# distributed-swarm/agent-tpu

Measured on AMD Instinct MI355X. Metric: classified rows/sec (whole node) map_classify BERT-base at 1/2/4/8 MI355X, higher is better.
Workload: dtype bf16; 1 GPU; model=bert-base, global_batch=1024, seq_len=128, parallelism=dp1, rccl_world_size=1, pg_world_size=1, distinct_devices=True, num_labels=2, topk=2, hipgraph=True, concurrent_batches=2, cu_split=False, weight_bytes=219212032, last_layer_cls_only=True

## Files before the change

agent_tpu_amd/csrc/bindings.cpp:

```cpp
#include <pybind11/numpy.h>
#include <pybind11/pybind11.h>
#include <pybind11/stl.h>

#include <algorithm>
#include <cstring>
#include <memory>
#include <string>
#include <vector>

#include "atpu/comm.h"
#include "atpu/common.h"
#include "atpu/csv.h"
#include "atpu/kernels.h"
#include "atpu/l2_prefetch.h"
#include "atpu/risk_stream.h"
#include "atpu/runtime.h"

namespace py = pybind11;
using namespace atpu;

namespace {

template <typename T>
T* P(uintptr_t p) {
// ... 130 lines not shown
      },
      "fin[m] = (rstd, rstd*mu) from StatsOut partials [slots][M][2]", py::arg("part"), py::arg("slots"),
      py::arg("M"), py::arg("K"), py::arg("eps"), py::arg("fin"), py::arg("stream"));
  m.def("trace_enabled", &trace_enabled, "roctx tracing active (MI355X_TRACE=1 and roctx loadable)");
  m.def("trace_push", [](const std::string& n) { trace_push(n.c_str()); });
  m.def("trace_pop", &trace_pop);
  m.def("trace_mark", [](const std::string& n) { trace_mark(n.c_str()); });
  m.def("gemm_splitk_splits", &gemm_splitk_splits, "split-K factor chosen for an [M,N,K] GEMM");
  m.def(
      "rand_fill",
      [](uintptr_t dst, int64_t n, bool f32, uint64_t seed, uint64_t sid, float scale0, int64_t n0, float scale1,
         uintptr_t stream) { rand_fill(P<void>(dst), n, f32, seed, sid, scale0, n0, scale1, S(stream)); },
      py::arg("dst"), py::arg("n"), py::arg("f32"), py::arg("seed"), py::arg("sid"), py::arg("scale0"), py::arg("n0"),
      py::arg("scale1"), py::arg("stream"), "seeded random init of a device tensor (atpu/rand.h)");
  m.def(
      "rand_fill_host",
      [](uintptr_t dst, int64_t n, bool f32, uint64_t seed, uint64_t sid, float scale0, int64_t n0, float scale1,
         int threads) {
        py::gil_scoped_release nogil;
        rand_fill_host(P<void>(dst), n, f32, seed, sid, scale0, n0, scale1, threads);
      },
      py::arg("dst"), py::arg("n"), py::arg("f32"), py::arg("seed"), py::arg("sid"), py::arg("scale0"), py::arg("n0"),
      py::arg("scale1"), py::arg("threads") = 8, "CPU twin of rand_fill (bit-identical values)");
  m.def("gemv_selected", &gemv_selected, py::arg("M"), py::arg("N"), py::arg("epi"),
        "true when gemm_bf16 runs this [M, N] problem / epilogue on the <= 4-row GEMV");
  m.def("batch_invariant", &batch_invariant, py::arg("set") = -1,
        "batch-invariant kernel selection (ATPU_BATCH_INVARIANT): 1 on, 0 off, -1 reads; returns the current");
  m.def("gemm_force_tile", &gemm_force_tile, py::arg("set") = -1, "GEMM kernel family override: 0 auto, 64, 128, 256");
  m.def("gemm_dec_mode", &gemm_dec_mode, py::arg("set") = -1,
        "skinny-M GEMM path: 1 = 64x64 multi-stage dec kernel, 0 = 128x128 split-K; returns the current");
  m.def("gemm_256_variant", &gemm_256_variant, py::arg("set") = -1,
        "256x256 GEMM schedule: 1 = 256p ping-pong, 3 = 256l persistent full-line epilogue, "
        "4 = 256n full-line + nt stores (default); set >= 0 switches, returns the current");
  m.def("cu_budget", &cu_budget, py::arg("set") = -1,
        "get/set the CU count persistent grids are sized for (0 = the device's; set it to the CU share of "
        "CU-masked streams)");
  m.def("num_cus", &num_cus, "CUs persistent grids are sized for");
  m.def("make_cu_mask_stream", &make_cu_mask_stream, py::arg("first_bit"), py::arg("nbits"),
        "create a HIP stream restricted to CU-mask bits [first_bit, first_bit+nbits) (bit i -> XCD i % 8); "
        "returns the hipStream_t as an int (wrap with torch.cuda.ExternalStream)");
  m.def("attention_persist_mode", &attention_persist_mode, py::arg("set") = -1,
        "packed BERT attention: 1 = persistent prefetching kernel (default), 0 = one item per workgroup");
  m.attr("EPI_BIAS") = static_cast<int>(kEpiBias);
  m.attr("EPI_GELU") = static_cast<int>(kEpiGelu);
  m.attr("EPI_TANH") = static_cast<int>(kEpiTanh);
  m.attr("EPI_RESIDUAL") = static_cast<int>(kEpiResidual);
  m.attr("EPI_RELU") = static_cast<int>(kEpiRelu);
  m.attr("EPI_OUT_F32") = static_cast<int>(kEpiOutF32);
  m.def(
      "cls_attend",
      [](uintptr_t g, uintptr_t fin, uintptr_t U, uintptr_t lens, uintptr_t Z, int B, int seq, int H, int heads,
         uintptr_t stream) {
        cls_attend(P<const bf16>(g), P<const float>(fin), P<const bf16>(U), P<const int32_t>(lens), P<bf16>(Z), B, seq,
                   H, heads, S(stream));
      },
      "[CLS] attention over raw hidden rows (K / V projection re-associated into U and the out-projection)",
      py::arg("g"), py::arg("fin"), py::arg("U"), py::arg("lens"), py::arg("Z"), py::arg("B"), py::arg("S"),
      py::arg("H"), py::arg("heads"), py::arg("stream"));
  m.def("decode_attention", [](uintptr_t q, int ldq, uintptr_t k, uintptr_t v, int ldkv, int seq_stride, int group,
                               uintptr_t lens, uintptr_t step_dev, uintptr_t hist, int hist_stride, uintptr_t bias,
                               int bias_stride, uintptr_t out, int ldo, int rows, int H, float scale, uintptr_t stream,
                               uintptr_t ws) {
    decode_attention(P<const bf16>(q), ldq, P<const bf16>(k), P<const bf16>(v), ldkv, seq_stride, group,
                     P<const int32_t>(lens), P<const int32_t>(step_dev), P<const int32_t>(hist), hist_stride,
                     P<const float>(bias), bias_stride, P<bf16>(out), ldo, rows, H, scale, S(stream), P<float>(ws));
  }, py::arg("q"), py::arg("ldq"), py::arg("k"), py::arg("v"), py::arg("ldkv"), py::arg("seq_stride"), py::arg("group"),
// ... 449 lines not shown
```

agent_tpu_amd/csrc/include/atpu/common.h:

```cpp
#pragma once

#include <hip/hip_runtime.h>

#include <cstdint>
#include <stdexcept>
#include <string>

namespace atpu {

typedef __bf16 bf16;
typedef __bf16 bf16x8 __attribute__((ext_vector_type(8)));
typedef __bf16 bf16x4 __attribute__((ext_vector_type(4)));
typedef float f32x4 __attribute__((ext_vector_type(4)));
typedef float f32x16 __attribute__((ext_vector_type(16)));

constexpr int kWave = 64;

#define ATPU_GLOBAL_AS __attribute__((address_space(1)))
#define ATPU_LDS_AS __attribute__((address_space(3)))

__device__ __forceinline__ void glds16(const void* gsrc, void* lds) {
  __builtin_amdgcn_global_load_lds((const ATPU_GLOBAL_AS void*)gsrc, (ATPU_LDS_AS void*)lds, 16, 0, 0);
}

__device__ __forceinline__ void wait_vmcnt0() { asm volatile("s_waitcnt vmcnt(0)" ::: "memory"); }

template <int CTRL>
__device__ __forceinline__ float dppf(float x) {
  return __int_as_float(__builtin_amdgcn_update_dpp(0, __float_as_int(x), CTRL, 0xF, 0xF, false));
}
constexpr int kDppMirror = 0x140, kDppHalfMirror = 0x141, kDppXor2 = 0x4E, kDppXor1 = 0xB1;

__device__ __forceinline__ float lane_rows_sum(float x);
__device__ __forceinline__ float lane_rows_max(float x);

__device__ __forceinline__ float wave_sum(float v) {
  v = lane_rows_sum(v);
  v += dppf<kDppMirror>(v);
  v += dppf<kDppHalfMirror>(v);
  v += dppf<kDppXor2>(v);
  return v + dppf<kDppXor1>(v);
}

__device__ __forceinline__ float wave_max(float v) {
  v = lane_rows_max(v);
  v = fmaxf(v, dppf<kDppMirror>(v));
  v = fmaxf(v, dppf<kDppHalfMirror>(v));
  v = fmaxf(v, dppf<kDppXor2>(v));
  return fmaxf(v, dppf<kDppXor1>(v));
}

__device__ __forceinline__ float lane_rows_sum(float x) {
  float a, b, c, d;
  asm volatile("v_mov_b32 %0, %2\n\tv_mov_b32 %1, %2\n\ts_nop 1\n\tv_permlane16_swap_b32 %0, %1"
               : "=&v"(a), "=&v"(b) : "v"(x));
// ... 166 lines not shown
    f32x2 phi;
    asm("v_pk_fma_f32 %0, %1, %2, %3 clamp" : "=v"(phi) : "v"(x[e]), "v"(p[e]), "v"(half));
    const f32x2 g = x[e] * phi;
    v[2 * e] = g[0];
    v[2 * e + 1] = g[1];
  }
}

__device__ __forceinline__ float gelu_poly1(float x) {
  constexpr int kDeg = 10;
  constexpr float kQ[kDeg + 1] = {1.536687613e-01f,  -7.178471889e-03f, 4.856055602e-04f, -3.426085095e-05f,
                                  2.347781901e-06f,  -1.526724844e-07f, 8.713541888e-09f, -4.079194205e-10f,
                                  2.366933385e-11f,  -1.725522828e-12f, 5.926992431e-14f};
  constexpr float kH = 1.056250000e+01f;
  const float w = fmaf(x, x, -kH);
  float p = kQ[kDeg];
#pragma unroll
  for (int k = kDeg - 1; k >= 0; --k) p = fmaf(p, w, kQ[k]);
  float phi;
  asm("v_fma_f32 %0, %1, %2, %3 clamp" : "=v"(phi) : "v"(x), "v"(p), "v"(0.5f));
  return x * phi;
}

__device__ __forceinline__ float bf2f(bf16 x) { return static_cast<float>(x); }
__device__ __forceinline__ bf16 f2bf(float x) { return static_cast<bf16>(x); }

typedef __bf16 bf16x2 __attribute__((ext_vector_type(2)));
typedef unsigned u32x4 __attribute__((ext_vector_type(4)));

__device__ __forceinline__ unsigned pack_bf16x2(float lo, float hi) {
  return __builtin_bit_cast(unsigned, bf16x2{f2bf(lo), f2bf(hi)});
}

__device__ __forceinline__ int xcd_remap(int b, int nblocks) {
  const int q = nblocks / 8, r = nblocks % 8, x = b % 8;
  return (x < r ? x * (q + 1) : r * (q + 1) + (x - r) * q) + b / 8;
}

}

#define ATPU_HIP_CHECK(expr)                                                              \
  do {                                                                                    \
    hipError_t _e = (expr);                                                               \
    if (_e != hipSuccess)                                                                 \
      throw std::runtime_error(std::string("HIP error ") + hipGetErrorString(_e) + " at " + \
                               __FILE__ + ":" + std::to_string(__LINE__));                \
  } while (0)

#define ATPU_CHECK(cond, msg)                                                   \
  do {                                                                          \
    if (!(cond)) throw std::invalid_argument(std::string("atpu: ") + (msg));    \
  } while (0)
```

agent_tpu_amd/csrc/include/atpu/kernels.h:

```cpp
#pragma once
#include <vector>

#include <hip/hip_runtime.h>

#include <cstdint>

namespace atpu {

typedef __bf16 bf16;

void rand_fill(void* dst, int64_t n, bool f32, uint64_t seed, uint64_t sid, float scale0, int64_t n0, float scale1,
               hipStream_t stream);

enum GemmEpilogue : int {
  kEpiBias = 1,
  kEpiGelu = 2,
  kEpiTanh = 4,
  kEpiResidual = 8,
  kEpiRelu = 16,
  kEpiOutF32 = 32,
  kEpiInNorm = 64,
  kEpiResNorm = 128,
  kEpiStatsOut = 256,
  kEpiKvScatter = 1024,
// ... 9 lines not shown
  const bf16* Bt = nullptr;
  int ldb = 0;
  bf16* C = nullptr;
  int ldc = 0;
  const float* bias = nullptr;
  const bf16* R = nullptr;
  int ldr = 0;
  int M = 0, N = 0, K = 0;
  int epi = 0;
  int splits = 1;
  float* ws = nullptr;
  const float* in_fin = nullptr;
  const float* colsum = nullptr;
  const float* res_fin = nullptr;
  const float* gamma = nullptr;
  float* part_out = nullptr;
  const float* in_part = nullptr;
  const float* res_part = nullptr;
  float rms_eps = 0.f;
  bf16* kv_cache = nullptr;
  int kv_ld = 0, kv_T = 0, kv_col0 = 0;
  const int32_t* kv_step = nullptr;
  const bf16* pf_w = nullptr;
  int pf_ld = 0, pf_k = 0, pf_n = 0;
  int pf_rpb = 16;
};
void gemm_bf16(const GemmArgs& g, hipStream_t stream);
bool gemv_selected(int M, int N, int epi);
int gemm_splitk_splits(int M, int N, int K);
int gemm_dec_mode(int set);
int batch_invariant(int set);
int gemm_force_tile(int set);
int gemm_256_variant(int set);
void gemm256h(const GemmArgs& g, int mode, hipStream_t stream);
void qkv_attention(const GemmArgs& g, const int32_t* lens, float scale, hipStream_t stream);
void cls_attend(const bf16* g, const float* fin, const bf16* U, const int32_t* lens, bf16* Z, int B, int S, int H,
                int heads, hipStream_t stream);

void quantize_rows_i8(const bf16* x, int ldx, int8_t* q, int ldq, float* scale, int rows, int K,
                      hipStream_t stream);
struct GemmI8Args {
  const int8_t* A = nullptr;
  int lda = 0;
  const float* a_scale = nullptr;
  const int8_t* Bt = nullptr;
  int ldb = 0;
  const float* b_scale = nullptr;
  bf16* C = nullptr;
  int ldc = 0;
  const float* bias = nullptr;
  const bf16* R = nullptr;
  int ldr = 0;
  int M = 0, N = 0, K = 0;
  int epi = 0;
  int32_t* acc_out = nullptr;
  int ldacc = 0;
};
void gemm_i8(const GemmI8Args& g, hipStream_t stream);
bool gemm_i8_ok(int M, int N, int K);
void layernorm_quant_i8(const bf16* x, const bf16* res, const float* gamma, const float* beta, bf16* out, int8_t* q,
                        float* scale, int rows, int N, float eps, hipStream_t stream);

int attention_persist_mode(int set);
int num_cus();
int cu_budget(int set);
int64_t make_cu_mask_stream(int first_bit, int nbits);
// ... 88 lines not shown
```

agent_tpu_amd/csrc/kernels/gemm_bf16.hip:

```cpp
#include "atpu/common.h"
#include "atpu/kernels.h"
#include "atpu/l2_prefetch.h"

#include <hip/hip_ext.h>

#include <algorithm>
#include <cstdlib>
#include <string>
#include <type_traits>

#ifndef ATPU_GEMM_SYNC_EPI
#define ATPU_GEMM_SYNC_EPI 1
#endif

namespace atpu {
namespace {

constexpr int kBK = 64;
constexpr int kRowBytes = kBK * 2;

__device__ __forceinline__ int swz(int row, int chunk) { return chunk ^ ((row >> 1) & 7); }

struct KvOut {
  bf16* cache = nullptr;
// ... 671 lines not shown
      const f32x2 s = f32x2{sum_lane_rows(s1[0] + s1[1]), sum_lane_rows(s2[0] + s2[1])};
      if (fc == 0) *reinterpret_cast<f32x2*>(ln.st + (wn * 256 + lrow) * 2) = s;
    }
#pragma unroll
    for (int j = 0; j < 4; ++j) {
      const unsigned p0 = pack_bf16x2(v[j][0], v[j][1]), p1 = pack_bf16x2(v[j][2], v[j][3]);
      typedef unsigned u32x2 __attribute__((ext_vector_type(2)));
      *reinterpret_cast<u32x2*>(scratch + frag_off(j)) = u32x2{p0, p1};
    }
    const u32x4 o0 = *reinterpret_cast<const u32x4*>(scratch + line_off0);
    const u32x4 o1 = *reinterpret_cast<const u32x4*>(scratch + line_off1);
    u32x4* cp = reinterpret_cast<u32x4*>(C + (row0 + i * 16 + lr) * ldc + col);
    u32x4* cp1 = reinterpret_cast<u32x4*>(C + (row0 + i * 16 + lr + 8) * ldc + col);
    if constexpr (NOST) {
      asm volatile("" ::"v"(o0), "v"(o1), "v"(cp), "v"(cp1));
    } else if constexpr (NT) {
      __builtin_nontemporal_store(o0, cp);
      __builtin_nontemporal_store(o1, cp1);
    } else {
      *cp = o0;
      *cp1 = o1;
    }
  }
}

struct LnFold {
  const float* in_fin;
  const float* colsum;
  const float* res_fin;
  const float* gamma;
  float* part_out;
};

template <int EPI, int DBG = 0, bool NT = false, bool LINE = false>
__global__ __launch_bounds__(512, 1) void gemm256s_kernel(
    const bf16* __restrict__ A, int lda, const bf16* __restrict__ Bt, int ldb, bf16* __restrict__ C, int ldc,
    const float* __restrict__ bias, const bf16* __restrict__ R, int ldr, int M, int N, int K, LnFold lf) {
  using namespace g2;
  constexpr int kImg = 256 * 128;
  constexpr int kEpiOps = kLineBlocks * kLineStoresPerBlock;
  static_assert(kEpiOps == 16, "epilogue store count changed: re-derive the relaxed waits");
  constexpr int kBiasOff = 2 * 2 * kImg;
  constexpr int kEpiOff = kBiasOff + 2 * 256 * 4;
  constexpr bool kIn = EPI & kEpiInNorm, kRes = EPI & kEpiResNorm, kSt = EPI & kEpiStatsOut;
  static_assert(!(kIn || kRes || kSt) || LINE, "LayerNorm folding needs the full-line epilogue");
  static_assert(!(kIn && (kRes || kSt)), "InNorm and ResNorm/StatsOut do not share one kernel (LDS budget)");
  constexpr int kXOff = kEpiOff + (LINE ? 8 * 2048 : 0);
  constexpr int kFinOff = kXOff;
  constexpr int kColOff = kFinOff + (kIn ? 4096 : kRes ? 2048 : 0);
  constexpr int kStOff = kColOff + ((kIn || kRes) ? 1024 : 0);
  constexpr int kLdsBytes = kStOff + (kSt ? 4 * 2048 : 0);
  static_assert(kLdsBytes <= 160 * 1024, "LDS budget");
  __shared__ __attribute__((aligned(16))) char lds[kLdsBytes];
  const int tid = threadIdx.x, lane = tid & 63;
  const int wave = __builtin_amdgcn_readfirstlane(tid >> 6);
  const int ntn = N / 256, ntm = (M + 255) / 256, ntiles = ntm * ntn;
  const int G = gridDim.x;
  const int wm = wave >> 2, wn = wave & 3;
  int v = blockIdx.x;
  if (v >= ntiles) return;

  const int spos = lane & 7;
  auto qrow = [&](int q, int ql) {
    return (q == 0 || q == 3) ? (ql & 63) + (ql >> 6) * 128 + (q == 3 ? 64 : 0)
                              : (ql & 31) + (ql >> 5) * 64 + (q == 2 ? 32 : 0);
  };
  int dst[4][2];
#pragma unroll
  for (int q = 0; q < 4; ++q)
#pragma unroll
    for (int i = 0; i < 2; ++i) dst[q][i] = (q == 0 || q == 3 ? 0 : kImg) + qrow(q, (i * 8 + wave) * 8) * 128;
  auto opaque_lane = [] {
    int l = __lane_id();
    asm volatile("" : "+v"(l));
    return l;
  };
  constexpr bool kFold = kIn || kRes || kSt;
  constexpr bool kSyncEpi = ATPU_GEMM_SYNC_EPI && !(DBG & 128);
  constexpr bool kInAcc = kIn && (DBG & 16);
  constexpr bool kPeel = kRes || kSt || (kIn && !kInAcc);
  constexpr bool kBiasAcc = (kRes || kSt) && (EPI & kEpiBias);
  const bf16* src[4][2];
  uint32_t soff[4][2];
  auto set_src = [&](int tm0, int tn0) {
    const int ln = kFold ? opaque_lane() : lane;
#pragma unroll
    for (int q = 0; q < 4; ++q)
#pragma unroll
      for (int i = 0; i < 2; ++i) {
        const int r = qrow(q, (i * 8 + wave) * 8 + (ln >> 3));
        const size_t e = (q == 0 || q == 3) ? (size_t)min(tm0 + r, M - 1) * lda + sw(r, ln & 7) * 8
                                            : (size_t)(tn0 + r) * ldb + sw(r, ln & 7) * 8;
        if constexpr (kFold) soff[q][i] = (uint32_t)(e * 2);
        else src[q][i] = ((q == 0 || q == 3) ? A : Bt) + e;
      }
  };
  auto stage = [&](int q, int kt, int buf) {
    char* base = lds + buf * 2 * kImg;
    const int koff = kt * 64;
    if constexpr (kFold) {
      const char* g = reinterpret_cast<const char*>((q == 0 || q == 3) ? A : Bt) + koff * 2;
      glds16(g + soff[q][0], base + dst[q][0]);
      glds16(g + soff[q][1], base + dst[q][1]);
    } else {
      glds16(src[q][0] + koff, base + dst[q][0]);
      glds16(src[q][1] + koff, base + dst[q][1]);
    }
  };

  const int fr = lane & 15, fc = lane >> 4;
  f32x4 acc[8][4];
  bf16x8 af[2][4], bl[2][2], br[2][2];
  auto read_a = [&](int buf, int qm) {
    const char* img = lds + buf * 2 * kImg;
#pragma unroll
    for (int ks = 0; ks < 2; ++ks)
#pragma unroll
      for (int i = 0; i < 4; ++i) {
        const int r = wm * 128 + qm * 64 + i * 16 + fr;
        af[ks][i] = *reinterpret_cast<const bf16x8*>(img + r * 128 + sw(r, ks * 4 + fc) * 16);
      }
  };
  auto read_b = [&](bf16x8 (&f)[2][2], int buf, int qn) {
    const char* img = lds + buf * 2 * kImg + kImg;
#pragma unroll
    for (int ks = 0; ks < 2; ++ks)
#pragma unroll
      for (int j = 0; j < 2; ++j) {
        const int r = wn * 64 + qn * 32 + j * 16 + fr;
        f[ks][j] = *reinterpret_cast<const bf16x8*>(img + r * 128 + sw(r, ks * 4 + fc) * 16);
      }
  };
  auto mma = [&](const bf16x8 (&bf)[2][2], int qm, int qn) {
#pragma unroll
    for (int ks = 0; ks < 2; ++ks)
#pragma unroll
// ... 7 lines not shown
  const int nk = K / 64;
  auto glds4 = [&](const float* ubase, char* ldst) {
    const uint32_t lo = (uint32_t)opaque_lane() * 4u;
    __builtin_amdgcn_global_load_lds((const ATPU_GLOBAL_AS void*)(reinterpret_cast<const char*>(ubase) + lo),
                                     (ATPU_LDS_AS void*)ldst, 4, 0, 0);
  };
  auto ln_stage = [&](int tm0, int tn0) {
    if constexpr (kRes || (kIn && !kInAcc)) {
      glds4((kRes ? lf.res_fin : lf.in_fin) + (size_t)tm0 * 2 + wave * 64, lds + kFinOff + wave * 256);
      glds4((kRes ? lf.gamma : lf.colsum) + tn0 + (wave & 3) * 64, lds + kColOff + (wave & 3) * 256);
    }
  };
  auto ln_stage_in = [&](int tm0, int tn0, int par) {
    if constexpr (kInAcc) {
      glds4(lf.in_fin + (size_t)tm0 * 2 + wave * 64, lds + kFinOff + par * 2048 + wave * 256);
      glds4(lf.colsum + tn0 + (wave & 3) * 64, lds + kColOff + (wave & 3) * 256);
    }
  };
  auto ln_flush = [&](int fm0, int fn0) {
    if constexpr (kSt) {
      const int l = opaque_lane();
      if (l < 32) {
        const int r = wave * 32 + l;
        f32x2 s = f32x2{0.f, 0.f};
#pragma unroll
        for (int w = 0; w < 4; ++w) s += *reinterpret_cast<const f32x2*>(lds + kStOff + (w * 256 + r) * 8);
        float* ub = lf.part_out + ((size_t)(fn0 >> 8) * M + fm0 + wave * 32) * 2;
        *reinterpret_cast<f32x2*>(reinterpret_cast<char*>(ub) + (uint32_t)l * 8u) = s;
      }
    }
  };
  int pm0 = 0, pn0 = 0;

  int tile = xcd_remap(v, ntiles);
  int m0 = (tile / ntn) * 256, n0 = (tile % ntn) * 256;
  set_src(m0, n0);
  if constexpr (kBiasAcc) glds4(bias + n0 + (wave & 3) * 64, lds + kBiasOff + (wave & 3) * 256);
  ln_stage_in(m0, n0, 0);
#pragma unroll
  for (int q = 0; q < 4; ++q) stage(q, 0, 0);
  asm volatile("s_waitcnt vmcnt(0)\n\ts_barrier" ::: "memory");
  if (wm == 1) __builtin_amdgcn_s_barrier();
  __builtin_amdgcn_sched_barrier(0);

#define ATPU_PS_SYNC_MMA(BF, QM, QN)                         \
  __builtin_amdgcn_sched_barrier(0);                        \
  __builtin_amdgcn_s_barrier();                             \
  asm volatile("s_waitcnt lgkmcnt(0)" ::: "memory");        \
  __builtin_amdgcn_sched_barrier(0);                        \
  __builtin_amdgcn_s_setprio(1);                            \
  mma(BF, QM, QN);                                          \
  __builtin_amdgcn_s_setprio(0);                            \
  __builtin_amdgcn_sched_barrier(0);                        \
  __builtin_amdgcn_s_barrier();                             \
  __builtin_amdgcn_sched_barrier(0)

  int buf = 0;
  int tile_par = 0;
  bool first = true;
  for (;;) {
    if constexpr (kBiasAcc) {
#pragma unroll
      for (int j = 0; j < 4; ++j) {
        const f32x4 b = *reinterpret_cast<const f32x4*>(lds + kBiasOff + (wn * 64 + j * 16 + fc * 4) * 4);
#pragma unroll
        for (int i = 0; i < 8; ++i) acc[i][j] = b;
      }
    } else if constexpr (kInAcc) {
      const int ol = opaque_lane();
      f32x4 c4[4];
#pragma unroll
      for (int j = 0; j < 4; ++j)
        c4[j] = *reinterpret_cast<const f32x4*>(lds + kColOff + (wn * 64 + j * 16 + (ol >> 4) * 4) * 4);
#pragma unroll
      for (int i = 0; i < 8; ++i) {
        const f32x2 f = *reinterpret_cast<const f32x2*>(lds + kFinOff + tile_par * 2048 +
                                                        (wm * 128 + i * 16 + (ol & 15)) * 8);
        const float nmu = -f[1] * __builtin_amdgcn_rcpf(f[0]);
#pragma unroll
        for (int j = 0; j < 4; ++j) acc[i][j] = c4[j] * nmu;
      }
    } else {
#pragma unroll
      for (int i = 0; i < 8; ++i)
#pragma unroll
        for (int j = 0; j < 4; ++j) acc[i][j] = f32x4{0.f, 0.f, 0.f, 0.f};
    }
    const int vn = v + G;
    const bool has_next = vn < ntiles;
    const int cm0 = m0, cn0 = n0;
    u32x4 pre[2][2];
    auto kstep = [&](int t, auto last_c, auto peel_c) {
      constexpr bool last = decltype(last_c)::value;
      constexpr int P = decltype(peel_c)::value;
      const bool is_t0 = P == -2 ? t == 0 : P == 0;
      const bool more = !last || has_next;
      int kn = t + 1;
      if (last && has_next) {
        tile = xcd_remap(vn, ntiles);
        m0 = (tile / ntn) * 256;
        n0 = (tile % ntn) * 256;
        set_src(m0, n0);
        kn = 0;
      }
      const bool relax = is_t0 && !first;
      read_a(buf, 0);
      read_b(bl, buf, 0);
      if constexpr (kBiasAcc) {
        if (last && has_next) glds4(bias + n0 + (wave & 3) * 64, lds + kBiasOff + (wave & 3) * 256);
      } else if ((EPI & kEpiBias) && is_t0) {
        const int bl_lane = (kIn || kRes || kSt) ? opaque_lane() : lane;
        __builtin_amdgcn_global_load_lds((const ATPU_GLOBAL_AS void*)(bias + cn0 + (wave & 3) * 64 + bl_lane),
                                         (ATPU_LDS_AS void*)(lds + kBiasOff + (tile_par * 256 + (wave & 3) * 64) * 4),
                                         4, 0, 0);
      }
      if constexpr (kInAcc) {
        if (last && has_next) ln_stage_in(m0, n0, tile_par ^ 1);
      }
      if constexpr (kPeel) {
        if constexpr (P == 1) {
          ln_stage(cm0, cn0);
          if (!first) ln_flush(pm0, pn0);
        }
      }
      if (more) {
        stage(0, kn, buf ^ 1);
        if (relax) asm volatile("s_waitcnt vmcnt(%0)" ::"n"(4 + kEpiOps) : "memory");
        else asm volatile("s_waitcnt vmcnt(4)" ::: "memory");
      } else {
        asm volatile("s_waitcnt vmcnt(2)" ::: "memory");
      }
      ATPU_PS_SYNC_MMA(bl, 0, 0);
      read_b(br, buf, 1);
      if (more) {
// ... 42 lines not shown
      for (int t = 0; t + 1 < nk; ++t) kstep(t, std::false_type{}, std::integral_constant<int, -2>{});
      kstep(nk - 1, std::true_type{}, std::integral_constant<int, -2>{});
    }
    if constexpr (kSyncEpi) {
      __builtin_amdgcn_sched_barrier(0);
      if (wm == 0) __builtin_amdgcn_s_barrier();
      __builtin_amdgcn_sched_barrier(0);
    }
    if constexpr (DBG & 1) {
#pragma unroll
      for (int i = 0; i < 8; ++i)
#pragma unroll
        for (int j = 0; j < 4; ++j) asm volatile("" ::"v"(acc[i][j]));
    } else {
      constexpr int kEpiRun0 = kBiasAcc ? (EPI & ~kEpiBias) : EPI;
      constexpr int kEpiRun = (DBG & 8) ? (kEpiRun0 & ~(kEpiInNorm | kEpiResNorm | kEpiStatsOut)) : kEpiRun0;
      if constexpr (LINE)
        epilogue_256_line<kEpiRun, NT, kInAcc, ((DBG >> 5) & 3), bool(DBG & 256)>(
            acc, cm0, cn0, wm, wn, (kIn || kRes || kSt) ? opaque_lane() : lane, C, ldc, R, ldr,
            reinterpret_cast<const float*>(lds + kBiasOff) + tile_par * 256, lds + kEpiOff + wave * 2048, pre,
            LnLds{reinterpret_cast<const float*>(lds + kFinOff + (kInAcc ? tile_par * 2048 : 0)),
                  reinterpret_cast<const float*>(lds + kColOff), reinterpret_cast<float*>(lds + kStOff)});
      else
        epilogue_256<EPI, true, (DBG >> 1), NT>(acc, cm0, cn0, wm, wn, lane, C, ldc, bias, R, ldr, M,
                                            reinterpret_cast<const float*>(lds + kBiasOff) + tile_par * 256);
    }
    if constexpr (kSyncEpi) {
      __builtin_amdgcn_sched_barrier(0);
      if (wm == 1) __builtin_amdgcn_s_barrier();
    }
    pm0 = cm0;
    pn0 = cn0;
    if (!has_next) break;
    v = vn;
    first = false;
    tile_par ^= 1;
  }
#undef ATPU_PS_SYNC_MMA
  if (wm == 0) __builtin_amdgcn_s_barrier();
  if constexpr (kSt) {
    asm volatile("s_waitcnt lgkmcnt(0)" ::: "memory");
    __builtin_amdgcn_s_barrier();
    ln_flush(pm0, pn0);
  }
}


}

static int g_cu_budget = 0;

int cu_budget(int set) {
  if (set >= 0) g_cu_budget = set;
  return g_cu_budget;
}

int num_cus() {
  static const int n = [] {
    int dev = 0, cus = 0;
    if (hipGetDevice(&dev) != hipSuccess || hipDeviceGetAttribute(&cus, hipDeviceAttributeMultiprocessorCount, dev) !=
                                                 hipSuccess)
      cus = 256;
    return cus > 0 ? cus : 256;
  }();
  return g_cu_budget > 0 ? std::min(g_cu_budget, n) : n;
}

int64_t make_cu_mask_stream(int first_bit, int nbits) {
  uint32_t mask[8] = {0, 0, 0, 0, 0, 0, 0, 0};
  for (int b = first_bit; b < first_bit + nbits && b < 256; ++b) mask[b / 32] |= 1u << (b % 32);
  hipStream_t s = nullptr;
  ATPU_HIP_CHECK(hipExtStreamCreateWithCUMask(&s, 8, mask));
  return reinterpret_cast<int64_t>(s);
}

namespace {

template <bool NT, bool LINE = false>
void launch_256s(const GemmArgs& g, hipStream_t s) {
  const int tiles = ((g.M + 255) / 256) * (g.N / 256);
  int nb = std::min(tiles, num_cus());
  if (nb >= 8) nb &= ~7;
  const LnFold lf{g.in_fin, g.colsum, g.res_fin, g.gamma, g.part_out};
#define ATPU_G256S(E)                                                                                          \
  case E:                                                                                                      \
    hipLaunchKernelGGL((gemm256s_kernel<E, 0, NT, LINE>), dim3(nb), dim3(512), 0, s, g.A, g.lda, g.Bt, g.ldb, g.C, g.ldc, \
                       g.bias, g.R, g.ldr, g.M, g.N, g.K, lf);                                                 \
    break;
  if constexpr (LINE) {
    switch (g.epi) {
      ATPU_G256S(kEpiBias | kEpiInNorm)
      ATPU_G256S(kEpiBias | kEpiInNorm | kEpiGelu)
      ATPU_G256S(kEpiBias | kEpiResidual | kEpiStatsOut)
      ATPU_G256S(kEpiBias | kEpiResidual | kEpiResNorm | kEpiStatsOut)
      default:
        break;
    }
    if (g.epi & (kEpiInNorm | kEpiResNorm | kEpiStatsOut)) return;
  }
  switch (g.epi) {
    ATPU_G256S(0)
    ATPU_G256S(kEpiBias)
    ATPU_G256S(kEpiBias | kEpiGelu)
    ATPU_G256S(kEpiBias | kEpiTanh)
    ATPU_G256S(kEpiBias | kEpiResidual)
    ATPU_G256S(kEpiResidual)
    ATPU_G256S(kEpiGelu)
    ATPU_G256S(kEpiRelu)
    default:
      throw std::invalid_argument("atpu: unsupported GEMM epilogue " + std::to_string(g.epi));
  }
#undef ATPU_G256S
}





template <int N>
__device__ __forceinline__ void wait_vmcnt() {
  asm volatile("s_waitcnt vmcnt(%0)" ::"n"(N) : "memory");
}

template <int EPI, int NJ>
__device__ __forceinline__ void dec_row_vals(const f32x4 (&acc)[NJ], int m, int nb, int fchunk, int N, float rstd,
                                             float rmu, float2 rf, bf16* __restrict__ C, int ldc,
                                             const float* __restrict__ bias, const bf16* __restrict__ R, int ldr,
                                             const KvOut& kvo, const LnDec& ln, int kv_pos, bf16x4 (&ov)[NJ]) {
#pragma unroll
  for (int j = 0; j < NJ; ++j) {
    const int n = nb + j * 16 + fchunk * 4;
    if (n >= N) continue;
    f32x4 v = acc[j];
    if constexpr (EPI & kEpiRowRms) v *= rstd;
    if constexpr (EPI & kEpiRowLn) {
      const f32x4 cs = *reinterpret_cast<const f32x4*>(ln.colsum + n);
#pragma unroll
      for (int e = 0; e < 4; ++e) v[e] = fmaf(v[e], rstd, -rmu * cs[e]);
    }
    if constexpr (EPI & kEpiBias) v += *reinterpret_cast<const f32x4*>(bias + n);
    if constexpr (EPI & kEpiGelu) {
#pragma unroll
      for (int e = 0; e < 4; ++e) v[e] = gelu_poly1(v[e]);
    }
    if constexpr (EPI & kEpiTanh) {
// ... 1083 lines not shown
```

agent_tpu_amd/csrc/kernels/qkv_attn.hip:

```cpp
#include "atpu/common.h"
#include "atpu/kernels.h"
#include "atpu/lds_ops.h"

#include <algorithm>

namespace atpu {
namespace {

constexpr int kHImgA = 256 * 128;
constexpr int kHImgB = 192 * 128;
constexpr int kHBuf = kHImgA + kHImgB;
constexpr int kHStores = 24;

__device__ __forceinline__ int hq_row(int q, int ql) {
  switch (q) {
    case 0: return (ql & 63) + (ql >> 6) * 128;
    case 3: return (ql & 63) + (ql >> 6) * 128 + 64;
    case 1: return (ql >> 5) * 48 + (ql & 31);
    default: return (ql >> 4) * 48 + 32 + (ql & 15);
  }
}
constexpr int hq_rounds(int q) { return q == 2 ? 1 : 2; }

constexpr int kAImg = kAttnImg;

template <int EPI, int MODE>
__global__ __launch_bounds__(512, 1) void gemm256h_kernel(const bf16* __restrict__ A, int lda,
                                                          const bf16* __restrict__ Bt, int ldb,
                                                          bf16* __restrict__ C, int ldc,
                                                          const float* __restrict__ bias,
                                                          const float* __restrict__ in_fin,
                                                          const float* __restrict__ colsum, int M, int N, int K,
                                                          const int32_t* __restrict__ lens, float scale) {
  constexpr bool kIn = EPI & kEpiInNorm;
  constexpr int kImgOff = kHBuf;
  constexpr int kBiasOff = MODE == 2 ? kImgOff + 6 * kAImg : 2 * kHBuf;
  constexpr int kFinOff = kBiasOff + 2 * 1024;
  constexpr int kColOff = kFinOff + 2048;
  constexpr int kLds = kColOff + 1024;
  constexpr int kEpiOps = MODE == 0 ? kHStores : MODE == 2 ? 4 : 0;
  constexpr int kLn1 = kIn ? 2 : 0;
  static_assert(kLds <= 160 * 1024, "LDS budget");
  __shared__ __attribute__((aligned(16))) char lds[kLds];
  const int tid = threadIdx.x, lane = tid & 63;
  const int wave = __builtin_amdgcn_readfirstlane(tid >> 6);
  const int wm = wave >> 2, wn = wave & 3;
  const int ntn = N / 192, ntiles = (M / 256) * ntn;
  const int G = gridDim.x;
  int v = blockIdx.x;
  if (v >= ntiles) return;

  auto opaque_lane = [] {
    int l = __lane_id();
    asm volatile("" : "+v"(l));
    return l;
  };
  int dst[4][2];
#pragma unroll
  for (int q = 0; q < 4; ++q)
#pragma unroll
    for (int i = 0; i < 2; ++i)
      dst[q][i] = (q == 0 || q == 3 ? 0 : kHImgA) + hq_row(q, (i * 8 + wave) * 8) * 128;
  uint32_t soff[4][2];
  auto set_src = [&](int tm0, int tn0) {
    const int ln = opaque_lane();
#pragma unroll
    for (int q = 0; q < 4; ++q)
#pragma unroll
      for (int i = 0; i < hq_rounds(q); ++i) {
        const int r = hq_row(q, (i * 8 + wave) * 8 + (ln >> 3));
        const size_t e = (q == 0 || q == 3) ? (size_t)(tm0 + r) * lda + hsw(r, ln & 7) * 8
                                            : (size_t)(tn0 + r) * ldb + hsw(r, ln & 7) * 8;
        soff[q][i] = (uint32_t)(e * 2);
      }
  };
  auto stage = [&](int q, int kt, int buf) {
    char* base = lds + buf * kHBuf;
    const char* g = reinterpret_cast<const char*>((q == 0 || q == 3) ? A : Bt) + kt * 128;
#pragma unroll
    for (int i = 0; i < hq_rounds(q); ++i) glds16(g + soff[q][i], base + dst[q][i]);
  };
  auto glds4 = [&](const float* ubase, int nvalid, char* ldst) {
    const int l = opaque_lane();
    __builtin_amdgcn_global_load_lds((const ATPU_GLOBAL_AS void*)(ubase + min(l, nvalid - 1)),
                                     (ATPU_LDS_AS void*)ldst, 4, 0, 0);
  };

  const int fr = lane & 15, fc = lane >> 4;
  f32x4 acc[8][3];
  bf16x8 af[2][4], b01[2][2], b2[2];
  auto read_a = [&](int buf, int qm) {
    const char* img = lds + buf * kHBuf;
#pragma unroll
    for (int ks = 0; ks < 2; ++ks)
#pragma unroll
      for (int i = 0; i < 4; ++i) {
        const int r = wm * 128 + qm * 64 + i * 16 + fr;
        af[ks][i] = *reinterpret_cast<const bf16x8*>(img + r * 128 + hsw(r, ks * 4 + fc) * 16);
      }
  };
  auto read_b01 = [&](int buf) {
    const char* img = lds + buf * kHBuf + kHImgA;
#pragma unroll
    for (int ks = 0; ks < 2; ++ks)
#pragma unroll
      for (int j = 0; j < 2; ++j) {
        const int r = wn * 48 + j * 16 + fr;
        b01[ks][j] = *reinterpret_cast<const bf16x8*>(img + r * 128 + hsw(r, ks * 4 + fc) * 16);
      }
  };
  auto read_b2 = [&](int buf) {
    const char* img = lds + buf * kHBuf + kHImgA;
#pragma unroll
// ... 168 lines not shown
    for (int ks = 0; ks < 4; ++ks) {
#pragma unroll
      for (int dt = 0; dt < 4; ++dt)
        o[1][dt] = __builtin_amdgcn_mfma_f32_16x16x32_bf16(vfrag(ks, dt), pf[1][ks],
                                                             ks ? o[1][dt] : f32x4{0.f, 0.f, 0.f, 0.f}, 0, 0, 0);
      o[1][4] = __builtin_amdgcn_mfma_f32_16x16x32_bf16(ones, pf[1][ks], ks ? o[1][4] : f32x4{0.f, 0.f, 0.f, 0.f}, 0, 0, 0);
    }
    __builtin_amdgcn_sched_barrier(0);
    char* ost = const_cast<char*>(qi) + wn * 32 * 128;
    const float inv1 = len > 0 && o[1][4][0] > 0.f ? 1.f / o[1][4][0] : 0.f;
#pragma unroll
    for (int dt = 0; dt < 4; ++dt) {
      unsigned x0 = xw[dt][0], x1 = xw[dt][1];
      unsigned y0 = pack_bf16x2(o[1][dt][0] * inv1, o[1][dt][1] * inv1);
      unsigned y1 = pack_bf16x2(o[1][dt][2] * inv1, o[1][dt][3] * inv1);
      swap16(x0, y0);
      swap16(x1, y1);
      const int ro = (fc & 1) * 16 + fr, ch = dt * 2 + (fc >> 1);
      *reinterpret_cast<u32x4*>(ost + ro * 128 + asw(ro, ch) * 16) = u32x4{x0, x1, y0, y1};
    }
    const int l2 = opaque_lane();
    const int lr = l2 >> 3, lc8 = l2 & 7;
    bf16* obase = C + (size_t)(tm0 + wm * 128 + wn * 32 + lr) * ldc + h * 64 + lc8 * 8;
#pragma unroll
    for (int hh = 0; hh < 4; ++hh) {
      const int ro = hh * 8 + lr;
      const u32x4 val = *reinterpret_cast<const u32x4*>(ost + ro * 128 + asw(ro, lc8) * 16);
      u32x4* dst = reinterpret_cast<u32x4*>(obase + (size_t)(hh * 8) * ldc);
      *dst = val;
    }
  };

  const int nk = K / 64;
  int tile = xcd_remap(v, ntiles);
  int m0 = (tile / ntn) * 256, n0 = (tile % ntn) * 192;
  set_src(m0, n0);
#pragma unroll
  for (int q = 0; q < 4; ++q) stage(q, 0, 0);
  asm volatile("s_waitcnt vmcnt(0)\n\ts_barrier" ::: "memory");
  if (wm == 1) __builtin_amdgcn_s_barrier();
  __builtin_amdgcn_sched_barrier(0);

#define ATPU_H_SYNC_MMA(MMA)                                \
  __builtin_amdgcn_sched_barrier(0);                        \
  __builtin_amdgcn_s_barrier();                             \
  asm volatile("s_waitcnt lgkmcnt(0)" ::: "memory");        \
  __builtin_amdgcn_sched_barrier(0);                        \
  __builtin_amdgcn_s_setprio(1);                            \
  MMA;                                                      \
  __builtin_amdgcn_s_setprio(0);                            \
  __builtin_amdgcn_sched_barrier(0);                        \
  __builtin_amdgcn_s_barrier();                             \
  __builtin_amdgcn_sched_barrier(0)

  int buf = 0, tile_par = 0;
  bool first = true;
  for (;;) {
#pragma unroll
    for (int i = 0; i < 8; ++i)
#pragma unroll
      for (int j = 0; j < 3; ++j) acc[i][j] = f32x4{0.f, 0.f, 0.f, 0.f};
    const int vn = v + G;
    const bool has_next = vn < ntiles;
    const int cm0 = m0, cn0 = n0;
    auto kstep = [&](int t, auto last_c, auto peel_c) {
      constexpr bool last = decltype(last_c)::value;
      constexpr int P = decltype(peel_c)::value;
      const bool more = !last || has_next;
      int kn = t + 1;
      if (last && has_next) {
        tile = xcd_remap(vn, ntiles);
        m0 = (tile / ntn) * 256;
        n0 = (tile % ntn) * 192;
        set_src(m0, n0);
        kn = 0;
      }
      const bool relax = P == 0 && !first;
      constexpr int kX = P == 0 ? 1 : (P == 1 ? kLn1 : 0);
      read_a(buf, 0);
      read_b01(buf);
      if (more) {
        stage(0, kn, buf ^ 1);
        stage(1, kn, buf ^ 1);
        if constexpr (P == 0) {
          glds4(bias + cn0 + wn * 48, 48, lds + kBiasOff + tile_par * 1024 + wn * 256);
        }
        if constexpr (P == 1 && kIn) {
          glds4(in_fin + (size_t)cm0 * 2 + wave * 64, 64, lds + kFinOff + wave * 256);
          glds4(colsum + cn0 + wn * 48, 48, lds + kColOff + wn * 256);
        }
        if (relax) asm volatile("s_waitcnt vmcnt(%0)" ::"n"(6 + kEpiOps + kX) : "memory");
        else asm volatile("s_waitcnt vmcnt(%0)" ::"n"(6 + kX) : "memory");
      } else {
        asm volatile("s_waitcnt vmcnt(2)" ::: "memory");
      }
      ATPU_H_SYNC_MMA(mma01(0));
      read_b2(buf);
      if (more) {
        stage(2, kn, buf ^ 1);
        if (relax) asm volatile("s_waitcnt vmcnt(%0)" ::"n"(5 + kEpiOps + kX) : "memory");
        else asm volatile("s_waitcnt vmcnt(%0)" ::"n"(5 + kX) : "memory");
      } else {
        asm volatile("s_waitcnt vmcnt(0)" ::: "memory");
      }
      ATPU_H_SYNC_MMA(mma2(0));
      read_a(buf, 1);
// ... 66 lines not shown
            *reinterpret_cast<u32x2*>(C + (size_t)(cm0 + wm * 128 + i * 16 + ofr) * ldc + cn0 + wn * 48 + j * 16 +
                                      ofc * 4) = u32x2{p0, p1};
          }
        }
      } else {
#pragma unroll
        for (int i = 0; i < 8; i += 2) {
#pragma unroll
          for (int j = 0; j < 3; ++j) {
            unsigned x0, x1, y0, y1;
            frag(i, j, x0, x1);
            frag(i + 1, j, y0, y1);
            swap16(x0, y0);
            swap16(x1, y1);
            const int cb = wn * 48 + j * 16, typ = cb >> 6;
            const int r = (i + (ofc & 1)) * 16 + ofr, ch = ((cb & 63) >> 3) + (ofc >> 1);
            *reinterpret_cast<u32x4*>(lds + kImgOff + (wm * 3 + typ) * kAImg + r * 128 + asw(r, ch) * 16) =
                u32x4{x0, x1, y0, y1};
          }
        }
      }
      if constexpr (MODE == 2) {
        asm volatile("s_waitcnt lgkmcnt(0)" ::: "memory");
        __builtin_amdgcn_s_barrier();
        __builtin_amdgcn_sched_barrier(0);
        attend(cm0, cn0 / 192, len);
        asm volatile("s_waitcnt lgkmcnt(0)" ::: "memory");
        __builtin_amdgcn_s_barrier();
      }
    }
    __builtin_amdgcn_sched_barrier(0);
    if (wm == 1) __builtin_amdgcn_s_barrier();
    if (!has_next) break;
    v = vn;
    first = false;
    tile_par ^= 1;
  }
#undef ATPU_H_SYNC_MMA
  if (wm == 0) __builtin_amdgcn_s_barrier();
}

}

static void launch_256h(const GemmArgs& g, int mode, const int32_t* lens, float scale, hipStream_t s) {
  ATPU_CHECK(g.N % 192 == 0 && g.M % 256 == 0 && g.K % 64 == 0 && g.K >= 256,
             "gemm256h: N % 192, M % 256 == 0, K % 64 == 0 and K >= 256");
  ATPU_CHECK(g.epi == kEpiBias || g.epi == (kEpiBias | kEpiInNorm), "gemm256h: epilogue bias or bias|InNorm");
  ATPU_CHECK(!(g.epi & kEpiInNorm) || (g.in_fin && g.colsum), "gemm256h: InNorm needs in_fin and colsum");
  ATPU_CHECK(g.bias && g.ldc % 4 == 0 && (reinterpret_cast<uintptr_t>(g.C) & 7) == 0, "gemm256h: bias, 8-B rows");
  ATPU_CHECK((size_t)g.M * g.lda * 2 < (1ull << 32) && (size_t)g.N * g.ldb * 2 < (1ull << 32),
             "gemm256h: A and Bt under 4 GiB (32-bit staging offsets)");
  ATPU_CHECK(mode >= 0 && mode <= 2, "gemm256h: mode 0 (store), 1 (timing only) or 2 (attention)");
  if (mode == 2) {
    ATPU_CHECK((g.K / 64) % 2 == 0, "qkv_attention: K / 64 must be even");
    ATPU_CHECK(lens && g.ldc % 8 == 0 && (reinterpret_cast<uintptr_t>(g.C) & 15) == 0,
               "qkv_attention: lens and 16-B aligned context rows");
  }
  const int tiles = (g.M / 256) * (g.N / 192);
  int nb = std::min(tiles, num_cus());
  if (nb >= 8) nb &= ~7;
#define ATPU_GH(E, MD)                                                                                          \
  hipLaunchKernelGGL((gemm256h_kernel<E, MD>), dim3(nb), dim3(512), 0, s, g.A, g.lda, g.Bt, g.ldb, g.C, g.ldc, \
                     g.bias, g.in_fin, g.colsum, g.M, g.N, g.K, lens, scale)
  if (g.epi & kEpiInNorm) {
    if (mode == 0) ATPU_GH(kEpiBias | kEpiInNorm, 0);
    else if (mode == 1) ATPU_GH(kEpiBias | kEpiInNorm, 1);
    else ATPU_GH(kEpiBias | kEpiInNorm, 2);
  } else {
    if (mode == 0) ATPU_GH(kEpiBias, 0);
    else if (mode == 1) ATPU_GH(kEpiBias, 1);
    else ATPU_GH(kEpiBias, 2);
  }
#undef ATPU_GH
  ATPU_HIP_CHECK(hipGetLastError());
}

void gemm256h(const GemmArgs& g, int mode, hipStream_t s) {
  ATPU_CHECK(mode == 0 || mode == 1, "gemm256h: mode 0 (store) or 1 (timing only, no epilogue)");
  launch_256h(g, mode, nullptr, 0.f, s);
}

void qkv_attention(const GemmArgs& g, const int32_t* lens, float scale, hipStream_t s) {
  launch_256h(g, 2, lens, scale, s);
}

}
```

Measured before the change: 52860 rows/s.

## Add XCD column-grouped tile walk and nt A-load policy to persistent GEMMs

Replaces the xcd_remap tile ordering in the persistent 256s and 256h GEMM kernels with a parameterised per-XCD walk. The walk can confine each XCD to a group of weight columns so the weights it reads stay resident in that XCD's L2. It also adds a template cache-policy option for the A-operand LDS-DMA loads (nt) and exposes both through env vars and bindings, plus host tools to inspect the walk. The defaults (cols=1, policy 0) are meant to reproduce the previous xcd_remap ordering with default loads, so the change mainly adds tuning knobs and carries a small cost of extra kernel arguments and index arithmetic.

```diff
diff --git a/agent_tpu_amd/csrc/bindings.cpp b/agent_tpu_amd/csrc/bindings.cpp
--- a/agent_tpu_amd/csrc/bindings.cpp
+++ b/agent_tpu_amd/csrc/bindings.cpp
@@ -186,6 +186,17 @@
   m.def("gemm_256_variant", &gemm_256_variant, py::arg("set") = -1,
         "256x256 GEMM schedule: 1 = 256p ping-pong, 3 = 256l persistent full-line epilogue, "
         "4 = 256n full-line + nt stores (default); set >= 0 switches, returns the current");
+  m.def("gemm_xcd_cols", &gemm_xcd_cols, py::arg("set") = -1,
+        "XCD tile walk of the persistent GEMMs: 0 = auto (column groups from the weight shape), 1 = the xcd_remap "
+        "walk, 2/4/8 = forced column groups; set >= 0 switches, returns the current (ATPU_GEMM_XCD_COLS)");
+  m.def("gemm_a_policy", &gemm_a_policy, py::arg("set") = -1,
+        "A-operand LDS-DMA cache policy of the persistent GEMMs: 0 = default loads, 1 = nt; set >= 0 switches, "
+        "returns the current (ATPU_GEMM_A_POLICY)");
+  m.def("gemm_walk_cols", &gemm_walk_cols, py::arg("ntn"), py::arg("tile_n"), py::arg("K"), py::arg("grid") = -1,
+        "column groups the launcher uses for a weight of ntn column tiles of tile_n rows and depth K "
+        "(1 below 8 workgroups and under cu_budget > 0)");
+  m.def("gemm_tile_walk", &gemm_tile_walk, py::arg("ntm"), py::arg("ntn"), py::arg("grid"), py::arg("cg"),
+        "host view of the persistent tile walk: the tile ids each of `grid` workgroups computes, in order");
   m.def("cu_budget", &cu_budget, py::arg("set") = -1,
         "get/set the CU count persistent grids are sized for (0 = the device's; set it to the CU share of "
         "CU-masked streams)");
diff --git a/agent_tpu_amd/csrc/include/atpu/common.h b/agent_tpu_amd/csrc/include/atpu/common.h
--- a/agent_tpu_amd/csrc/include/atpu/common.h
+++ b/agent_tpu_amd/csrc/include/atpu/common.h
@@ -21,6 +21,11 @@
 
 __device__ __forceinline__ void glds16(const void* gsrc, void* lds) {
   __builtin_amdgcn_global_load_lds((const ATPU_GLOBAL_AS void*)gsrc, (ATPU_LDS_AS void*)lds, 16, 0, 0);
+}
+
+template <int POL>
+__device__ __forceinline__ void glds16_pol(const void* gsrc, void* lds) {
+  __builtin_amdgcn_global_load_lds((const ATPU_GLOBAL_AS void*)gsrc, (ATPU_LDS_AS void*)lds, 16, 0, POL);
 }
 
 __device__ __forceinline__ void wait_vmcnt0() { asm volatile("s_waitcnt vmcnt(0)" ::: "memory"); }
@@ -253,9 +258,32 @@
   return __builtin_bit_cast(unsigned, bf16x2{f2bf(lo), f2bf(hi)});
 }
 
-__device__ __forceinline__ int xcd_remap(int b, int nblocks) {
+__host__ __device__ __forceinline__ int xcd_remap(int b, int nblocks) {
   const int q = nblocks / 8, r = nblocks % 8, x = b % 8;
   return (x < r ? x * (q + 1) : r * (q + 1) + (x - r) * q) + b / 8;
+}
+
+struct XcdWalk {
+  int row0, col0, ncol, off, count;
+};
+
+__host__ __device__ __forceinline__ XcdWalk xcd_walk_init(int x, int ntm, int ntn, int cg) {
+  if (cg <= 1) {
+    const int nt = ntm * ntn, q = nt / 8, r = nt % 8;
+    const int start = x < r ? x * (q + 1) : r * (q + 1) + (x - r) * q;
+    return XcdWalk{start / ntn, 0, ntn, start % ntn, q + (x < r ? 1 : 0)};
+  }
+  const int per = 8 / cg, g = x / per, j = x % per;
+  const int q = ntm / per, r = ntm % per, ncol = ntn / cg;
+  return XcdWalk{j < r ? j * (q + 1) : r * (q + 1) + (j - r) * q, g * ncol, ncol, 0, (q + (j < r ? 1 : 0)) * ncol};
+}
+
+__host__ __device__ __forceinline__ int xcd_col_walk(int v, int ntm, int ntn, int cg) {
+  const XcdWalk w = xcd_walk_init(v % 8, ntm, ntn, cg);
+  const int l = v / 8;
+  if (l >= w.count) return -1;
+  const int p = w.off + l, r = p / w.ncol;
+  return (w.row0 + r) * ntn + w.col0 + (p - r * w.ncol);
 }
 
 }
diff --git a/agent_tpu_amd/csrc/include/atpu/kernels.h b/agent_tpu_amd/csrc/include/atpu/kernels.h
--- a/agent_tpu_amd/csrc/include/atpu/kernels.h
+++ b/agent_tpu_amd/csrc/include/atpu/kernels.h
@@ -65,6 +65,10 @@
 int batch_invariant(int set);
 int gemm_force_tile(int set);
 int gemm_256_variant(int set);
+int gemm_xcd_cols(int set);
+int gemm_a_policy(int set);
+int gemm_walk_cols(int ntn, int tile_n, int K, int grid);
+std::vector<std::vector<int>> gemm_tile_walk(int ntm, int ntn, int grid, int cg);
 void gemm256h(const GemmArgs& g, int mode, hipStream_t stream);
 void qkv_attention(const GemmArgs& g, const int32_t* lens, float scale, hipStream_t stream);
 void cls_attend(const bf16* g, const float* fin, const bf16* U, const int32_t* lens, bf16* Z, int B, int S, int H,
diff --git a/agent_tpu_amd/csrc/kernels/gemm_bf16.hip b/agent_tpu_amd/csrc/kernels/gemm_bf16.hip
--- a/agent_tpu_amd/csrc/kernels/gemm_bf16.hip
+++ b/agent_tpu_amd/csrc/kernels/gemm_bf16.hip
@@ -727,10 +727,10 @@
   float* part_out;
 };
 
-template <int EPI, int DBG = 0, bool NT = false, bool LINE = false>
+template <int EPI, int DBG = 0, bool NT = false, bool LINE = false, int APOL = 0>
 __global__ __launch_bounds__(512, 1) void gemm256s_kernel(
     const bf16* __restrict__ A, int lda, const bf16* __restrict__ Bt, int ldb, bf16* __restrict__ C, int ldc,
-    const float* __restrict__ bias, const bf16* __restrict__ R, int ldr, int M, int N, int K, LnFold lf) {
+    const float* __restrict__ bias, const bf16* __restrict__ R, int ldr, int M, int N, int K, LnFold lf, int cg) {
   using namespace g2;
   constexpr int kImg = 256 * 128;
   constexpr int kEpiOps = kLineBlocks * kLineStoresPerBlock;
@@ -749,11 +749,12 @@
   __shared__ __attribute__((aligned(16))) char lds[kLdsBytes];
   const int tid = threadIdx.x, lane = tid & 63;
   const int wave = __builtin_amdgcn_readfirstlane(tid >> 6);
-  const int ntn = N / 256, ntm = (M + 255) / 256, ntiles = ntm * ntn;
-  const int G = gridDim.x;
+  const int ntn = N / 256, ntm = (M + 255) / 256;
+  const XcdWalk xw = xcd_walk_init(blockIdx.x % 8, ntm, ntn, cg);
+  const int wstep = max((int)gridDim.x / 8, 1);
   const int wm = wave >> 2, wn = wave & 3;
-  int v = blockIdx.x;
-  if (v >= ntiles) return;
+  int wl = blockIdx.x / 8;
+  if (wl >= xw.count) return;
 
   const int spos = lane & 7;
   auto qrow = [&](int q, int ql) {
@@ -795,8 +796,16 @@
     const int koff = kt * 64;
     if constexpr (kFold) {
       const char* g = reinterpret_cast<const char*>((q == 0 || q == 3) ? A : Bt) + koff * 2;
-      glds16(g + soff[q][0], base + dst[q][0]);
-      glds16(g + soff[q][1], base + dst[q][1]);
+      if (q == 0 || q == 3) {
+        glds16_pol<APOL>(g + soff[q][0], base + dst[q][0]);
+        glds16_pol<APOL>(g + soff[q][1], base + dst[q][1]);
+      } else {
+        glds16(g + soff[q][0], base + dst[q][0]);
+        glds16(g + soff[q][1], base + dst[q][1]);
+      }
+    } else if (q == 0 || q == 3) {
+      glds16_pol<APOL>(src[q][0] + koff, base + dst[q][0]);
+      glds16_pol<APOL>(src[q][1] + koff, base + dst[q][1]);
     } else {
       glds16(src[q][0] + koff, base + dst[q][0]);
       glds16(src[q][1] + koff, base + dst[q][1]);
@@ -870,8 +879,13 @@
   };
   int pm0 = 0, pn0 = 0;
 
-  int tile = xcd_remap(v, ntiles);
-  int m0 = (tile / ntn) * 256, n0 = (tile % ntn) * 256;
+  int m0, n0;
+  auto walk_tile = [&](int l) {
+    const int p = xw.off + l, r = p / xw.ncol;
+    m0 = (xw.row0 + r) * 256;
+    n0 = (xw.col0 + p - r * xw.ncol) * 256;
+  };
+  walk_tile(wl);
   set_src(m0, n0);
   if constexpr (kBiasAcc) glds4(bias + n0 + (wave & 3) * 64, lds + kBiasOff + (wave & 3) * 256);
   ln_stage_in(m0, n0, 0);
@@ -924,8 +938,8 @@
 #pragma unroll
         for (int j = 0; j < 4; ++j) acc[i][j] = f32x4{0.f, 0.f, 0.f, 0.f};
     }
-    const int vn = v + G;
-    const bool has_next = vn < ntiles;
+    const int wln = wl + wstep;
+    const bool has_next = wln < xw.count;
     const int cm0 = m0, cn0 = n0;
     u32x4 pre[2][2];
     auto kstep = [&](int t, auto last_c, auto peel_c) {
@@ -935,9 +949,7 @@
       const bool more = !last || has_next;
       int kn = t + 1;
       if (last && has_next) {
-        tile = xcd_remap(vn, ntiles);
-        m0 = (tile / ntn) * 256;
-        n0 = (tile % ntn) * 256;
+        walk_tile(wln);
         set_src(m0, n0);
         kn = 0;
       }
@@ -1046,7 +1058,7 @@
     pm0 = cm0;
     pn0 = cn0;
     if (!has_next) break;
-    v = vn;
+    wl = wln;
     first = false;
     tile_par ^= 1;
   }
@@ -1067,6 +1079,61 @@
 int cu_budget(int set) {
   if (set >= 0) g_cu_budget = set;
   return g_cu_budget;
+}
+
+constexpr int kXcdColsDefault = 1;
+constexpr int kAPolicyDefault = 0;
+constexpr int64_t kXcdWeightBudget = 2500000;
+
+int gemm_xcd_cols(int set) {
+  static int v = [] {
+    const char* f = std::getenv("ATPU_GEMM_XCD_COLS");
+    const int e = f ? std::atoi(f) : kXcdColsDefault;
+    return (e == 0 || e == 1 || e == 2 || e == 4 || e == 8) ? e : kXcdColsDefault;
+  }();
+  if (set >= 0) {
+    ATPU_CHECK(set == 0 || set == 1 || set == 2 || set == 4 || set == 8,
+               "gemm_xcd_cols: 0 (auto), 1 (xcd_remap walk) or a grouping of 2, 4, 8");
+    v = set;
+  }
+  return v;
+}
+
+int gemm_a_policy(int set) {
+  static int v = [] {
+    const char* f = std::getenv("ATPU_GEMM_A_POLICY");
+    const int e = f ? std::atoi(f) : kAPolicyDefault;
+    return (e == 0 || e == 1) ? e : kAPolicyDefault;
+  }();
+  if (set >= 0) {
+    ATPU_CHECK(set == 0 || set == 1, "gemm_a_policy: 0 (default loads) or 1 (nt)");
+    v = set;
+  }
+  return v;
+}
+
+int gemm_walk_cols(int ntn, int tile_n, int K, int grid) {
+  if ((grid >= 0 && grid < 8) || g_cu_budget > 0) return 1;
+  const int mode = gemm_xcd_cols(-1);
+  if (mode >= 1) return (ntn % mode == 0) ? mode : 1;
+  for (int cg = 1; cg <= 8; cg *= 2)
+    if (ntn % cg == 0 && (int64_t)(ntn / cg) * tile_n * K * 2 <= kXcdWeightBudget) return cg;
+  return 1;
+}
+
+std::vector<std::vector<int>> gemm_tile_walk(int ntm, int ntn, int grid, int cg) {
+  ATPU_CHECK(ntm > 0 && ntn > 0 && grid > 0, "gemm_tile_walk: positive sizes");
+  ATPU_CHECK((cg == 1 || cg == 2 || cg == 4 || cg == 8) && ntn % cg == 0, "gemm_tile_walk: cg in {1,2,4,8}, ntn % cg == 0");
+  ATPU_CHECK(grid % 8 == 0 || (grid < 8 && grid == ntm * ntn && cg == 1),
+             "gemm_tile_walk: grid % 8 == 0, or one workgroup per tile below 8");
+  std::vector<std::vector<int>> out(grid);
+  for (int b = 0; b < grid; ++b)
+    for (int v = b;; v += grid) {
+      const int t = xcd_col_walk(v, ntm, ntn, cg);
+      if (t < 0) break;
+      out[b].push_back(t);
+    }
+  return out;
 }
 
 int num_cus() {
@@ -1096,10 +1163,15 @@
   int nb = std::min(tiles, num_cus());
   if (nb >= 8) nb &= ~7;
   const LnFold lf{g.in_fin, g.colsum, g.res_fin, g.gamma, g.part_out};
-#define ATPU_G256S(E)                                                                                          \
-  case E:                                                                                                      \
-    hipLaunchKernelGGL((gemm256s_kernel<E, 0, NT, LINE>), dim3(nb), dim3(512), 0, s, g.A, g.lda, g.Bt, g.ldb, g.C, g.ldc, \
-                       g.bias, g.R, g.ldr, g.M, g.N, g.K, lf);                                                 \
+  const int cg = gemm_walk_cols(g.N / 256, 256, g.K, nb);
+  const bool a_nt = gemm_a_policy(-1) == 1;
+#define ATPU_G256S_POL(E, POL)                                                                                 \
+  hipLaunchKernelGGL((gemm256s_kernel<E, 0, NT, LINE, POL>), dim3(nb), dim3(512), 0, s, g.A, g.lda, g.Bt, g.ldb, g.C, \
+                     g.ldc, g.bias, g.R, g.ldr, g.M, g.N, g.K, lf, cg)
+#define ATPU_G256S(E)                    \
+  case E:                                \
+    if (a_nt) ATPU_G256S_POL(E, 2);      \
+    else ATPU_G256S_POL(E, 0);           \
     break;
   if constexpr (LINE) {
     switch (g.epi) {
@@ -1125,6 +1197,7 @@
       throw std::invalid_argument("atpu: unsupported GEMM epilogue " + std::to_string(g.epi));
   }
 #undef ATPU_G256S
+#undef ATPU_G256S_POL
 }
 
 
diff --git a/agent_tpu_amd/csrc/kernels/qkv_attn.hip b/agent_tpu_amd/csrc/kernels/qkv_attn.hip
--- a/agent_tpu_amd/csrc/kernels/qkv_attn.hip
+++ b/agent_tpu_amd/csrc/kernels/qkv_attn.hip
@@ -24,14 +24,14 @@
 
 constexpr int kAImg = kAttnImg;
 
-template <int EPI, int MODE>
+template <int EPI, int MODE, int APOL = 0>
 __global__ __launch_bounds__(512, 1) void gemm256h_kernel(const bf16* __restrict__ A, int lda,
                                                           const bf16* __restrict__ Bt, int ldb,
                                                           bf16* __restrict__ C, int ldc,
                                                           const float* __restrict__ bias,
                                                           const float* __restrict__ in_fin,
                                                           const float* __restrict__ colsum, int M, int N, int K,
-                                                          const int32_t* __restrict__ lens, float scale) {
+                                                          const int32_t* __restrict__ lens, float scale, int cg) {
   constexpr bool kIn = EPI & kEpiInNorm;
   constexpr int kImgOff = kHBuf;
   constexpr int kBiasOff = MODE == 2 ? kImgOff + 6 * kAImg : 2 * kHBuf;
@@ -45,10 +45,11 @@
   const int tid = threadIdx.x, lane = tid & 63;
   const int wave = __builtin_amdgcn_readfirstlane(tid >> 6);
   const int wm = wave >> 2, wn = wave & 3;
-  const int ntn = N / 192, ntiles = (M / 256) * ntn;
-  const int G = gridDim.x;
-  int v = blockIdx.x;
-  if (v >= ntiles) return;
+  const int ntn = N / 192;
+  const XcdWalk xw = xcd_walk_init(blockIdx.x % 8, M / 256, ntn, cg);
+  const int wstep = max((int)gridDim.x / 8, 1);
+  int wl = blockIdx.x / 8;
+  if (wl >= xw.count) return;
 
   auto opaque_lane = [] {
     int l = __lane_id();
@@ -78,7 +79,10 @@
     char* base = lds + buf * kHBuf;
     const char* g = reinterpret_cast<const char*>((q == 0 || q == 3) ? A : Bt) + kt * 128;
 #pragma unroll
-    for (int i = 0; i < hq_rounds(q); ++i) glds16(g + soff[q][i], base + dst[q][i]);
+    for (int i = 0; i < hq_rounds(q); ++i) {
+      if (q == 0 || q == 3) glds16_pol<APOL>(g + soff[q][i], base + dst[q][i]);
+      else glds16(g + soff[q][i], base + dst[q][i]);
+    }
   };
   auto glds4 = [&](const float* ubase, int nvalid, char* ldst) {
     const int l = opaque_lane();
@@ -313,8 +317,13 @@
   };
 
   const int nk = K / 64;
-  int tile = xcd_remap(v, ntiles);
-  int m0 = (tile / ntn) * 256, n0 = (tile % ntn) * 192;
+  int m0, n0;
+  auto walk_tile = [&](int l) {
+    const int p = xw.off + l, r = p / xw.ncol;
+    m0 = (xw.row0 + r) * 256;
+    n0 = (xw.col0 + p - r * xw.ncol) * 192;
+  };
+  walk_tile(wl);
   set_src(m0, n0);
 #pragma unroll
   for (int q = 0; q < 4; ++q) stage(q, 0, 0);
@@ -341,8 +350,8 @@
     for (int i = 0; i < 8; ++i)
 #pragma unroll
       for (int j = 0; j < 3; ++j) acc[i][j] = f32x4{0.f, 0.f, 0.f, 0.f};
-    const int vn = v + G;
-    const bool has_next = vn < ntiles;
+    const int wln = wl + wstep;
+    const bool has_next = wln < xw.count;
     const int cm0 = m0, cn0 = n0;
     auto kstep = [&](int t, auto last_c, auto peel_c) {
       constexpr bool last = decltype(last_c)::value;
@@ -350,9 +359,7 @@
       const bool more = !last || has_next;
       int kn = t + 1;
       if (last && has_next) {
-        tile = xcd_remap(vn, ntiles);
-        m0 = (tile / ntn) * 256;
-        n0 = (tile % ntn) * 192;
+        walk_tile(wln);
         set_src(m0, n0);
         kn = 0;
       }
@@ -485,7 +492,7 @@
     __builtin_amdgcn_sched_barrier(0);
     if (wm == 1) __builtin_amdgcn_s_barrier();
     if (!has_next) break;
-    v = vn;
+    wl = wln;
     first = false;
     tile_par ^= 1;
   }
@@ -512,9 +519,16 @@
   const int tiles = (g.M / 256) * (g.N / 192);
   int nb = std::min(tiles, num_cus());
   if (nb >= 8) nb &= ~7;
-#define ATPU_GH(E, MD)                                                                                          \
-  hipLaunchKernelGGL((gemm256h_kernel<E, MD>), dim3(nb), dim3(512), 0, s, g.A, g.lda, g.Bt, g.ldb, g.C, g.ldc, \
-                     g.bias, g.in_fin, g.colsum, g.M, g.N, g.K, lens, scale)
+  const int cg = gemm_walk_cols(g.N / 192, 192, g.K, nb);
+  const bool a_nt = gemm_a_policy(-1) == 1;
+#define ATPU_GH_POL(E, MD, POL)                                                                                      \
+  hipLaunchKernelGGL((gemm256h_kernel<E, MD, POL>), dim3(nb), dim3(512), 0, s, g.A, g.lda, g.Bt, g.ldb, g.C, g.ldc, \
+                     g.bias, g.in_fin, g.colsum, g.M, g.N, g.K, lens, scale, cg)
+#define ATPU_GH(E, MD)                 \
+  do {                                 \
+    if (a_nt) ATPU_GH_POL(E, MD, 2);   \
+    else ATPU_GH_POL(E, MD, 0);        \
+  } while (0)
   if (g.epi & kEpiInNorm) {
     if (mode == 0) ATPU_GH(kEpiBias | kEpiInNorm, 0);
     else if (mode == 1) ATPU_GH(kEpiBias | kEpiInNorm, 1);
@@ -525,6 +539,7 @@
     else ATPU_GH(kEpiBias, 2);
   }
 #undef ATPU_GH
+#undef ATPU_GH_POL
   ATPU_HIP_CHECK(hipGetLastError());
 }
 
```

Measured after the change: 52940 rows/s (median of 6 runs). About the same (+0.2%).
